# thodan/epos

Measured on AMD Instinct MI355X. Metric: images/sec end-to-end (CNN+PnP-RANSAC), YCB-V 640x480, higher is better.
Workload: dtype f32

## Files before the change

epos_amd/_lib.py:

```python
import ctypes
import os

from epos_amd import build as _build

c_f32p = ctypes.POINTER(ctypes.c_float)
c_f64p = ctypes.POINTER(ctypes.c_double)
c_i32p = ctypes.POINTER(ctypes.c_int32)
c_i64p = ctypes.POINTER(ctypes.c_int64)
c_u64p = ctypes.POINTER(ctypes.c_uint64)
vp = ctypes.c_void_p


class EposError(RuntimeError):
  pass


class PointwiseArgs(ctypes.Structure):
  _fields_ = [
      ('A', vp), ('lda', ctypes.c_int64),
      ('Wp', vp), ('bias', vp),
      ('R', vp), ('ldr', ctypes.c_int64),
      ('C', vp), ('ldc', ctypes.c_int64),
      ('M', ctypes.c_int32), ('N', ctypes.c_int32), ('K', ctypes.c_int32),
      ('relu', ctypes.c_int32), ('relu_in', ctypes.c_int32),
# ... 137 lines not shown
      ('use_prosac', ctypes.c_int32),
      ('lo_iters', ctypes.c_int32),
      ('gc_sweeps', ctypes.c_int32),
      ('pearl_iters', ctypes.c_int32),
  ]


class PnpRansacParams(ctypes.Structure):
  _fields_ = [
      ('iterations_count', ctypes.c_int32),
      ('min_point_number', ctypes.c_int32),
      ('reprojection_error', ctypes.c_double),
      ('confidence', ctypes.c_double),
  ]


SYMBOLS = {
    'epos_abi_version': (ctypes.c_int, []),
    'epos_last_error': (ctypes.c_char_p, []),
    'epos_device_count': (ctypes.c_int, []),
    'epos_clock_probe': (ctypes.c_int, [ctypes.c_void_p, ctypes.c_int, ctypes.c_void_p]),
    'epos_pack_pointwise_weights': (ctypes.c_int64,
                                    [vp, ctypes.c_int, ctypes.c_int, vp]),
    'epos_pack_pointwise_weights_split': (ctypes.c_int64,
                                          [vp, ctypes.c_int, ctypes.c_int, vp]),
    'epos_pack_pointwise_weights_h2': (ctypes.c_int64,
                                       [vp, ctypes.c_int, ctypes.c_int, vp]),
    'epos_absmax_f32': (ctypes.c_int, [vp, ctypes.c_int64, ctypes.c_int64,
                                       ctypes.c_int64, vp, vp]),
    'epos_amax_clear': (ctypes.c_int, [vp, ctypes.c_int64, vp]),
    'epos_pointwise_conv_f32': (ctypes.c_int,
                                [ctypes.POINTER(PointwiseArgs), vp]),
    'epos_pointwise_conv_grouped_f32': (ctypes.c_int, [
        ctypes.POINTER(PointwiseArgs), ctypes.c_int, vp]),
    'epos_conv3x3_f32': (ctypes.c_int, [ctypes.POINTER(Conv3x3Args), ctypes.c_void_p]),
    'epos_depthwise3x3_f32': (ctypes.c_int,
                              [ctypes.POINTER(DepthwiseArgs), vp]),
    'epos_separable_conv_f32': (ctypes.c_int, [ctypes.POINTER(SepConvArgs), vp]),
    'epos_set_h2_narrow_tile_limit': (ctypes.c_int, [ctypes.c_int]),
    'epos_im2col3x3_f32': (ctypes.c_int, [ctypes.POINTER(Im2colArgs), vp]),
    'epos_im2col_f32': (ctypes.c_int, [ctypes.POINTER(Im2colKArgs), vp]),
    'epos_global_avg_pool_partial_f32': (ctypes.c_int, [
        vp, ctypes.c_int64, vp, ctypes.c_int, ctypes.c_int, ctypes.c_int, ctypes.c_int, vp]),
    'epos_global_avg_pool_f32': (ctypes.c_int, [
        vp, ctypes.c_int64, vp, ctypes.c_int, ctypes.c_int, ctypes.c_int, vp]),
    'epos_resize_bilinear_f32': (ctypes.c_int, [
        vp, ctypes.c_int64, vp, ctypes.c_int64, ctypes.c_int, ctypes.c_int,
        ctypes.c_int, ctypes.c_int, ctypes.c_int, ctypes.c_int, vp]),
    'epos_maxpool3x3_s2_f32': (ctypes.c_int, [
        vp, ctypes.c_int64, vp, ctypes.c_int64, ctypes.c_int, ctypes.c_int,
        ctypes.c_int, ctypes.c_int, vp]),
    'epos_subsample_f32': (ctypes.c_int, [
        vp, ctypes.c_int64, vp, ctypes.c_int64, ctypes.c_int, ctypes.c_int,
        ctypes.c_int, ctypes.c_int, ctypes.c_int, vp]),
    'epos_add_relu_f32': (ctypes.c_int, [vp, vp, vp, ctypes.c_int64, vp]),
    'epos_softmax_groups_f32': (ctypes.c_int,
                                [vp, ctypes.c_int64, ctypes.c_int, vp]),
    'epos_u8_to_f32': (ctypes.c_int, [vp, vp, ctypes.c_int64, vp]),
    'epos_scatter_blocks_f32': (ctypes.c_int, [vp, vp, vp, ctypes.c_int64, ctypes.c_int, vp]),
    'epos_argmax_i64': (ctypes.c_int, [
        vp, ctypes.c_int64, vp, ctypes.c_int64, ctypes.c_int, vp]),
    'epos_softmax_slots_f32': (ctypes.c_int, [
        vp, vp, ctypes.c_int, ctypes.c_int, ctypes.c_int, ctypes.c_int, vp]),
    'epos_corr_count': (ctypes.c_int, [
        vp, vp, vp, ctypes.c_int, ctypes.c_int, ctypes.c_int, ctypes.c_int,
        ctypes.c_int, ctypes.c_float, ctypes.c_float, vp, vp, vp, vp, vp]),
# ... 100 lines not shown
```

epos_amd/csrc/pointwise_gemm.h:

```cpp
#pragma once
#include <stdlib.h>

#include <mutex>
#include <type_traits>

#include "common.h"

namespace epos {

struct Fp32MfmaRef {
  int (*dma)(const EposPointwiseArgs* args, int count, hipStream_t s, const int* conv_cin,
             const int* conv_rate);
  int (*staged)(const EposPointwiseArgs* args, int count, hipStream_t s);
};
Fp32MfmaRef& fp32_mfma_ref();
int launch_grouped_split(const EposPointwiseArgs* args, int count, hipStream_t s,
                         const int* conv_cin = nullptr, const int* conv_rate = nullptr);
bool split_eligible(const EposPointwiseArgs* args, int count);
int launch_grouped_h2(const EposPointwiseArgs* args, int count, hipStream_t s,
                      const int* conv_cin = nullptr, const int* conv_rate = nullptr);
bool h2_eligible(const EposPointwiseArgs* args, int count);

namespace {

struct LdsAttrOnce {
  std::mutex mu;
  bool set[16] = {};
};
inline int ensure_dynamic_lds(LdsAttrOnce& once, const void* kern, int bytes, const char* what) {
  int dev = 0;
  if (hipGetDevice(&dev) != hipSuccess || dev < 0 || dev >= 16) {
    set_error("%s: no current device", what);
    return EPOS_E_INVALID;
  }
  std::lock_guard<std::mutex> lock(once.mu);
  if (once.set[dev]) return EPOS_OK;
  const int rc = check_hip(hipFuncSetAttribute(kern, hipFuncAttributeMaxDynamicSharedMemorySize,
                                               bytes), what);
  if (!rc) once.set[dev] = true;
  return rc;
}

constexpr int BN = 128;
constexpr int BK = 32;
constexpr int LDS_A_ROW = BK + 4;
constexpr int LDS_B_TILE = (BK / 4) * BN * 4;
constexpr int THREADS = 256;
constexpr int MAX_GROUP = 8;

typedef float f32x16 __attribute__((ext_vector_type(16)));

struct GroupedArgs {
  EposPointwiseArgs p[MAX_GROUP];
  int tile_start[MAX_GROUP + 1];
// ... 135 lines not shown
```

epos_amd/csrc/pointwise_gemm.hip:

```cpp
#include "pointwise_gemm.h"

namespace epos {

Fp32MfmaRef& fp32_mfma_ref() {
  static Fp32MfmaRef hooks = {nullptr, nullptr};
  return hooks;
}

namespace {

int no_fp32_mfma(const char* what) {
  set_error("%s: this problem brings neither fp16-pair (Wh + a bound for A) nor bf16 x 6 (Ws) "
            "weights, and this build of libepos_hip.so carries no fp32-MFMA kernel (they are "
            "test-only since round 6: libepos_hip_ref.so, `python -m epos_amd.build --ref`, "
            "EPOS_HIP_LIB=<that file>)", what);
  return EPOS_E_INVALID;
}

constexpr int GEMV_SLICES = 16;

__global__ __launch_bounds__(64 * GEMV_SLICES) void pointwise_gemv_f32(EposPointwiseArgs p,
                                                                       int npad) {
  __shared__ float part[GEMV_SLICES][64];
  const int t = threadIdx.x;
// ... 73 lines not shown
  const int64_t npad = round_up(N, BN);
  const int64_t total = kg * npad * 4;
  if (!dst) return total;
  for (int64_t q = 0; q < kg; ++q)
    for (int64_t n = 0; n < npad; ++n)
      for (int e = 0; e < 4; ++e) {
        const int64_t k = q * 4 + e;
        dst[(q * npad + n) * 4 + e] =
            (k < K && n < N) ? w_kn[k * static_cast<int64_t>(N) + n] : 0.f;
      }
  return total;
}

static int grouped_impl(const EposPointwiseArgs* args, int count, void* stream);

extern "C" int epos_pointwise_conv_grouped_f32(const EposPointwiseArgs* args,
                                               int count, void* stream) {
  using namespace epos;
  EPOS_REQUIRE(args && count >= 1 && count <= MAX_GROUP, "1..8 problems per group");
  for (int i = 0; i < count; ++i) {
    const EposPointwiseArgs& a = args[i];
    EPOS_REQUIRE(a.reserved0 == 0, "EposPointwiseArgs.reserved0 must be 0 (ABI 7)");
    if (a.col_sums)
      EPOS_REQUIRE(!a.R && a.N % 4 == 0 && a.col_ld % 4 == 0 && a.col_ld >= a.N &&
                       (reinterpret_cast<uintptr_t>(a.col_sums) & 15) == 0 &&
                       (a.ldc & 3) == 0 && (reinterpret_cast<uintptr_t>(a.C) & 15) == 0 &&
                       h2_eligible(args, count),
                   "col_sums needs the fp16-pair kernel (Wh, a bound for A), no residual, "
                   "N, ldc, col_ld multiples of 4 and 16-byte aligned C / col_sums");
  }
  return grouped_impl(args, count, stream);
}

static int grouped_impl(const EposPointwiseArgs* args, int count, void* stream) {
  using namespace epos;
  hipStream_t s = static_cast<hipStream_t>(stream);
  for (int i = 0; i < count; ++i) {
    const int rc = validate(&args[i]);
    if (rc) return rc;
    EPOS_REQUIRE((args[i].relu_in != 0) == (args[0].relu_in != 0) &&
                 (args[i].R != nullptr) == (args[0].R != nullptr),
                 "problems of one group must agree on relu_in / residual");
  }
  if (count == 1 && args[0].M <= 8 && args[0].sub == 1) {
    const int npad = static_cast<int>(round_up(args[0].N, BN));
    hipLaunchKernelGGL(pointwise_gemv_f32, dim3(npad / 64, args[0].M),
                       dim3(64 * GEMV_SLICES), 0, s, args[0], npad);
    return launch_status("pointwise_gemv_f32");
  }
  if (h2_eligible(args, count)) return launch_grouped_h2(args, count, s);
  for (int i = 0; i < count; ++i)
    EPOS_REQUIRE(!args[i].a_presplit,
                 "a pre-split A operand needs the fp16-pair kernel (every problem of the "
                 "group with Wh; EPOS_GEMM_H2 / EPOS_GEMM_SPLIT not 0)");
  if (split_eligible(args, count)) return launch_grouped_split(args, count, s);
  const Fp32MfmaRef& ref = fp32_mfma_ref();
  static const int use_dma = [] {
    const char* e = getenv("EPOS_GEMM_DMA");
    return e ? atoi(e) : -1;
  }();
  if (args[0].relu_in == 0 && use_dma != 0 && ref.dma)
    return ref.dma(args, count, s, nullptr, nullptr);
  if (ref.staged) return ref.staged(args, count, s);
  return no_fp32_mfma("epos_pointwise_conv_grouped_f32");
}

// ... 57 lines not shown
```

epos_amd/csrc/pointwise_gemm_h2.hip:

```cpp
#include <string.h>

#include <mutex>
#include <utility>

#include "h2_scale.h"
#include "pointwise_gemm.h"

namespace epos {
namespace {

typedef _Float16 f16x8 __attribute__((ext_vector_type(8)));
typedef unsigned u32x4 __attribute__((ext_vector_type(4)));
typedef float h2_f32x4 __attribute__((ext_vector_type(4)));

#ifdef EPOS_GEMM_TRACE
__device__ uint64_t* g_h2_trace = nullptr;
#define H2_STAMP(i) do { if (g_h2_trace && t == 0) g_h2_trace[8 * static_cast<uint64_t>(blockIdx.x) + (i)] = wall_clock64(); } while (0)
#else
#define H2_STAMP(i) do { } while (0)
#endif
constexpr int RING_DEVICES = 16;
constexpr int H2_BM = 128, H2_BN = 128, H2_BK = 16;
constexpr int H2_W_BYTES = H2_BK * H2_BN * 4;
constexpr int H2_A_BYTES = H2_BM * H2_BK * 4;
// ... 784 lines not shown
}

void set_tn_div(GroupedArgs& g, int i) {
  const unsigned d = static_cast<unsigned>(g.tiles_n[i] > 0 ? g.tiles_n[i] : 1);
  unsigned l = 0;
  while ((1ull << l) < d) ++l;
  g.tn_mul[i] = static_cast<unsigned>(((1ull << 32) * ((1ull << l) - d)) / d + 1);
  g.tn_sh1[i] = l > 0 ? 1 : 0;
  g.tn_sh2[i] = l > 0 ? l - 1 : 0;
}

constexpr int RING_SLOTS = 256;
unsigned* ring_slot(hipStream_t s) {
  static std::mutex mu;
  static unsigned* base[RING_DEVICES] = {};
  static unsigned next[RING_DEVICES] = {};
  int dev = 0;
  if (hipGetDevice(&dev) != hipSuccess || dev < 0 || dev >= RING_DEVICES) return nullptr;
  {
    std::lock_guard<std::mutex> lock(mu);
    if (!base[dev] && capturing(s)) return nullptr;
    if (!base[dev] &&
        hipMalloc(reinterpret_cast<void**>(&base[dev]),
                  sizeof(unsigned) * EPOS_AMAX_WORDS * RING_SLOTS) != hipSuccess) {
      base[dev] = nullptr;
      return nullptr;
    }
  }
  const unsigned i = __atomic_fetch_add(&next[dev], 1u, __ATOMIC_RELAXED) % RING_SLOTS;
  return base[dev] + static_cast<size_t>(i) * EPOS_AMAX_WORDS;
}

}

bool h2_eligible(const EposPointwiseArgs* args, int count) {
  static const int mode = [] {
    const char* e = getenv("EPOS_GEMM_H2");
    const char* sp = getenv("EPOS_GEMM_SPLIT");
    if (sp && atoi(sp) == 0) return 0;
    return e ? atoi(e) : 1;
  }();
  if (mode == 0) return false;
  for (int i = 0; i < count; ++i) {
    const EposPointwiseArgs& a = args[i];
    if (!a.Wh || a.relu_in != 0 || a.M <= 8 || (a.K & 3) != 0 || (a.lda & 3) != 0 ||
        (reinterpret_cast<uintptr_t>(a.A) & 15) != 0)
      return false;
    if (a.a_presplit && !a.a_amax) return false;
    const int64_t rows = a.sub > 1 ? static_cast<int64_t>(a.M) / (static_cast<int64_t>(a.Ho) * a.Wo) *
                                         a.Hi * a.Wi
                                   : a.M;
    if (rows * a.lda * 4 >= (1LL << 32)) return false;
  }
  return true;
}

int& narrow_limit() {
  static int v = [] {
    const char* e = getenv("EPOS_H2_BN64_MAX_TILES");
    return e ? atoi(e) : 100;
  }();
  return v;
}

int launch_grouped_h2(const EposPointwiseArgs* args, int count, hipStream_t s,
                      const int* conv_cin, const int* conv_rate) {
// ... 220 lines not shown
```

epos_amd/net.py:

```python
import ctypes
import os

import numpy as np
import torch

from epos_amd import _lib
from epos_amd import weights as W
from epos_amd.net_modes import Bf16Mode, Fp32Mode, _ptr

XCEPTION_BN_EPS = 1e-3
HEAD_BN_EPS = 1e-5
RESNET_BN_EPS = 1e-5
MODES = {'fp32': Fp32Mode, 'bf16': Bf16Mode}
PRECISIONS = tuple(MODES)
PREPROCESS = {None: _lib.PREPROCESS_NONE, 'unit_range': _lib.PREPROCESS_UNIT_RANGE,
              'sub_mean': _lib.PREPROCESS_SUB_MEAN}
PREPROCESS_EXPR = {'unit_range': 'preprocess(input)', 'sub_mean': 'submean(input)'}


def scale_dimension(dim, scale):
  return int((float(dim) - 1.0) * scale + 1.0)


_CAPTURE_STREAMS = {}
# ... 407 lines not shown
    mode.resize('decoder/resize', proj, 256, dcat, ldd, eh, ew, dh, dw_, 256)
    self._set_expr(dcat, self._expr_of(proj) if (eh, ew) == (dh, dw_) else
                   'resize(%s,%dx%d)' % (self._expr_of(proj), dh, dw_), 0, 256)
    m_dec = B * dh * dw_
    self._conv1x1('decoder/feature_projection0', HEAD_BN_EPS, ll, 0, lc, m_dec, lc, dcat,
                  256, ldd, relu=True)
    mode.concat_bound(dcat, proj)
    self.decoder_concat = dcat[..., :304]
    x, c = dcat, 304
    for j in range(2):
      scope = 'decoder/decoder_conv%d' % j
      d, _, _ = self._depthwise(scope + '_depthwise', x, self._ld(x), dh, dw_, c, 1, 1,
                                HEAD_BN_EPS, False, True)
      y = self._abuf(B, dh, dw_, 256)
      self._conv1x1(scope + '_pointwise', HEAD_BN_EPS, d, 0, self._ld(d), m_dec, c, y, 0,
                    256, relu=True)
      x, c = y, 256
    self.decoder_out = x
    self.out_h, self.out_w = dh, dw_

    self.logits = {}
    grp = []
    self._n_trunk_ops = len(self.ops)
    for name, ch in sorted(W.outputs_to_num_channels(
        self.num_objs, self.num_frags).items()):
      buf = self._empty(B, dh, dw_, ch)
      self._conv1x1('logits/' + name, None, x, 0, 256, m_dec, 256, buf, 0, ch, relu=False,
                    group=grp, track_out=False)
      self.logits[name] = buf
    if os.environ.get('EPOS_HEAD_NT_STORES', '1') == '1':
      for g in grp:
        g[1].c_stream = 1
    oname, oargs, oflops = [g for g in grp if g[0].endswith(W.PRED_OBJ_CONF)][0][:3]
    mode.flush(grp)
    self._obj_head_op = (oname, mode.obj_head(oname, oargs))
    self._obj_head_flops = oflops
    self._decoder_x = x

    obj = self.logits[W.PRED_OBJ_CONF]
    frag = self.logits[W.PRED_FRAG_CONF]
    self.obj_label = self._empty(B, dh, dw_, dtype=torch.int64)
    O, F = self.num_objs, self.num_frags
    softmax = self._fn('epos_softmax_groups_f32')
    self.post_ops = [
        ('softmax_obj', self._call('softmax_obj', softmax, (_ptr(obj), m_dec, O + 1))),
        ('softmax_frag', self._call('softmax_frag', softmax, (_ptr(frag), m_dec * O, F))),
        ('argmax', self._call('argmax', self._fn('epos_argmax_i64'),
                              (_ptr(obj), O + 1, _ptr(self.obj_label), m_dec, O + 1)))]
    eo = self._expr_of(self.logits[W.PRED_OBJ_CONF])
    ef = self._expr_of(self.logits[W.PRED_FRAG_CONF])
    el = self._expr_of(self.logits[W.PRED_FRAG_LOC])
    self.trace_outputs = {
        W.PRED_OBJ_CONF: {'expr': 'softmax(%s)' % eo, 'shape': [B, dh, dw_, O + 1]},
        W.PRED_OBJ_LABEL: {'expr': 'argmax(softmax(%s))' % eo, 'shape': [B, dh, dw_]},
        W.PRED_FRAG_CONF: {'expr': 'softmax(reshape(%s,%s))' % (ef, [O, F]),
                           'shape': [B, dh, dw_, O, F]},
        W.PRED_FRAG_LOC: {'expr': 'reshape(%s,%s)' % (el, [O, F, 3]),
                          'shape': [B, dh, dw_, O, F, 3]}}
    mode.finish()

  def algorithmic_bytes(self, dense_heads=True):
    total = self._glue_bytes
    for a_bytes, rest, a_id in self.op_io.values():
      total += self._dw_reads.get(a_id, a_bytes) + rest
    if not dense_heads:
      total -= 4 * self.B * self.out_h * self.out_w * (4 * self.num_objs * self.num_frags)
    return total
# ... 151 lines not shown
```

epos_amd/net_modes.py:

```python
import ctypes
import os

import numpy as np
import torch

from epos_amd import _lib
from epos_amd import weights as W


def _ptr(t, offset_elems=0):
  return ctypes.c_void_p(t.data_ptr() + offset_elems * t.element_size())


def _fold(w_kn, scale, kmult):
  k, n = w_kn.shape
  w = w_kn.astype(np.float32) * scale[None, :].astype(np.float32)
  kpad = -(-k // kmult) * kmult
  if kpad != k:
    w = np.concatenate([w, np.zeros((kpad - k, n), np.float32)], 0)
  return np.ascontiguousarray(w)


def _pack(fn, w, dtype):
  src = w.ctypes.data_as(ctypes.c_void_p)
  total = fn(src, w.shape[0], w.shape[1], None)
  if total <= 0:
    return None
  dst = np.empty(total, dtype)
  fn(src, w.shape[0], w.shape[1], dst.ctypes.data_as(ctypes.c_void_p))
  return dst


def _bias(bias, n, mult):
  b = np.zeros(-(-n // mult) * mult, np.float32)
  b[:n] = bias
  return b


class Fp32Mode(object):

  dtype, line = torch.float32, 32
  MAX_SLOTS = 512

  def __init__(self, net):
    self.net = net
    fn = net._fn
    self.gemm = fn('epos_pointwise_conv_grouped_f32')
    self.gemm1 = fn('epos_pointwise_conv_f32')
    self.dw = fn('epos_depthwise3x3_f32')
    self.conv3x3 = fn('epos_conv3x3_f32')
    self.im2col3x3 = fn('epos_im2col3x3_f32')
    self.im2col_k = fn('epos_im2col_f32')
    self.absmax = fn('epos_absmax_f32')
    self.amax_clear = fn('epos_amax_clear')
    self.avg_pool = fn('epos_global_avg_pool_f32')
    self.avg_pool_partial = fn('epos_global_avg_pool_partial_f32')
    self.resize_fn = fn('epos_resize_bilinear_f32')
    self.subsample = fn('epos_subsample_f32')
    self.add_relu = fn('epos_add_relu_f32')
    self.maxpool = fn('epos_maxpool3x3_s2_f32')
    self.pack_plain = fn('epos_pack_pointwise_weights')
    self.pack_split = fn('epos_pack_pointwise_weights_split')
    self.pack_h2 = fn('epos_pack_pointwise_weights_h2')
    self._amax_table = torch.zeros(self.MAX_SLOTS * _lib.AMAX_WORDS, dtype=torch.int32,
                                   device=net.dev)
    self._slot_count = ctypes.c_int64(0)
    self._bounds = {}
    self.use_h2 = (os.environ.get('EPOS_GEMM_H2', '1') != '0' and
                   os.environ.get('EPOS_GEMM_SPLIT', '1') != '0')
    self.use_presplit = self.use_h2 and os.environ.get('EPOS_H2_PRESPLIT', '1') == '1'
    self._dw_h2 = {}
    self.h2_layers, self.h2_refused, self.presplit_layers = [], [], []
    self._last_pw = None
    self._first_im2col = None

  @property
  def _n_slots(self):
    return self._slot_count.value

  def _new_slot(self):
    i = self._slot_count.value
# ... 66 lines not shown
                ldr=0, sub=1, ho=0, wo=0, hi=0, wi=0, group=None, track_out=True):
    net = self.net
    ab = self._bounds.get(id(a)) if self.use_h2 else None
    wp, bp, ws, wh, kpad = self._weights(name, conv, ab is not None and m > 8)
    n = conv[0].shape[1]
    assert kpad == k or (kpad > k and lda >= kpad), (name, k, kpad, lda)
    dwa = self._dw_h2.pop(id(a), None)
    presplit = False
    if dwa is not None:
      presplit = wh is not None and sub == 1 and a_off == 0
      dwa.y_h2 = int(presplit)
      if presplit:
        self.presplit_layers.append(name)
    track = track_out and m > 8 and (res is None or ldr % 4 == 0)
    cslot = self._out_slot(c, n, ldc, c_off) if track else None
    h = wh is not None
    args = _lib.PointwiseArgs(
        A=_ptr(a, a_off), lda=lda, Wp=_ptr(wp), bias=_ptr(bp),
        R=_ptr(res, res_off) if res is not None else None, ldr=ldr,
        C=_ptr(c, c_off), ldc=ldc, M=m, N=n, K=kpad, relu=int(relu), sub=sub,
        Ho=ho, Wo=wo, Hi=hi, Wi=wi, Ws=_ptr(ws), Wh=_ptr(wh) if h else None,
        a_amax=self._slot_ptr(ab[0]) if h else None,
        a_amax2=self._slot_ptr(ab[1]) if h else None,
        a_gain=ab[2] if h else 0.0, a_bias=ab[3] if h else 0.0,
        a_presplit=int(presplit), c_amax=self._slot_ptr(cslot))
    nbytes = 4 * (m * k + k * n + m * n + (m * n if res is not None else 0))
    net.op_io[name] = (4 * m * k, nbytes - 4 * m * k, id(a))
    if group is not None:
      group.append((name, args, 2 * m * n * k, nbytes))
      return
    net._launch(name, self.gemm, (args, 1), 'gemm', 2 * m * n * k, nbytes)
    self._last_pw = (c, args, h and res is None and c_off == 0 and n % 4 == 0)

  def flush(self, group):
    for kind in sorted({g[1].a_presplit for g in group}):
      part = [g for g in group if g[1].a_presplit == kind]
      arr = (_lib.PointwiseArgs * len(part))(*[g[1] for g in part])
      self.net._launch('+'.join(g[0] for g in part), self.gemm, (arr, len(part)), 'gemm',
                       sum(g[2] for g in part), sum(g[3] for g in part))
    del group[:]

  def depthwise(self, name, x, y, gain, bias0, flops, nbytes, **fields):
    xb = self._bounds.get(id(x))
    if xb is not None:
      self._set_bound(y, xb[0], xb[1], gain * (xb[2] if xb[2] else 1.0), gain * xb[3] + bias0)
    args = _lib.DepthwiseArgs(**fields)
    yb = self._bounds.get(id(y))
    if yb is not None and self.use_presplit:
      args.y_h2 = 1
      args.x_amax, args.x_amax2 = self._slot_ptr(yb[0]), self._slot_ptr(yb[1])
      args.gain, args.bias0 = yb[2], yb[3]
      self._dw_h2[id(y)] = args
    self.net._launch(name, self.dw, (args,), 'dw', flops, nbytes)

  def dense_conv(self, name, x, y, hi, wi, cin, ho, wo, kk, stride, rate, pad, preprocess,
                 conv):
    net, B = self.net, self.net.B
    cout = y.shape[3]
    k = kk * kk * cin
    if kk == 3 and cin % 32 == 0 and preprocess == _lib.PREPROCESS_NONE:
      xb = self._bounds.get(id(x))
      wp, bp, ws, wh, _ = self._weights(name, conv, xb is not None and xb[1] is None and
                                        xb[2] == 0.0)
      yslot = self._out_slot(y, cout, cout)
      args = _lib.Conv3x3Args(X=_ptr(x), ldx=cin, Wp=_ptr(wp), bias=_ptr(bp), Y=_ptr(y),
                              ldy=cout, B=B, H=hi, W=wi, Cin=cin, Cout=cout, stride=stride,
                              rate=rate, relu=1, Ws=_ptr(ws),
                              Wh=_ptr(wh) if wh is not None else None,
                              x_amax=self._slot_ptr(xb[0]) if wh is not None else None,
                              y_amax=self._slot_ptr(yslot))
      net._launch(name, self.conv3x3, (args,), 'gemm', 2 * B * ho * wo * cout * k,
# ... 134 lines not shown
    args = _lib.PointwiseBf16Args(
        A=_ptr(a, a_off) if a is not None else None, lda=lda, Wp=_ptr(wp), bias=_ptr(bp),
        R=_ptr(res, res_off) if res is not None else None, ldr=ldr,
        C=_ptr(c, c_off), ldc=ldc, M=m, N=n, K=kpad, relu=int(relu), sub=sub,
        Ho=ho, Wo=wo, Hi=hi, Wi=wi, c_f32=int(c.dtype == torch.float32), c_stream=0)
    nbytes = (2 * (m * k + k * n) + c.element_size() * m * n +
              (2 * m * n if res is not None else 0))
    net.op_io[name] = (2 * m * k, nbytes - 2 * m * k, id(a))
    if group is not None:
      group.append((name, args, 2 * m * n * k, nbytes))
      return args
    net._launch(name, self.gemm, (args, 1), 'gemm', 2 * m * n * k, nbytes)
    return args

  def _pointwise_f32(self, name, a, lda, m, k, conv, c, ldc, relu):
    net = self.net
    w_kn, scale, bias = conv
    n = w_kn.shape[1]
    kpad = -(-k // 4) * 4
    assert kpad == k, (name, k)
    if net.dry_run:
      wp, bp, ws = net._empty(1), net._empty(1), net._empty(1)
    else:
      w = _fold(w_kn, scale, 4)
      wp, bp = net._dev(_pack(self.pack_plain, w, np.float32)), net._dev(_bias(bias, n, 128))
      ws = net._dev(_pack(self.pack_split, w, np.uint8))
    args = _lib.PointwiseArgs(A=_ptr(a), lda=lda, Wp=_ptr(wp), bias=_ptr(bp), C=_ptr(c),
                              ldc=ldc, M=m, N=n, K=kpad, relu=int(relu), sub=1, Ws=_ptr(ws))
    nbytes = 4 * (m * k + k * n + m * n)
    net.op_io[name] = (4 * m * k, nbytes - 4 * m * k, id(a))
    net._launch(name, self.gemm_f32, (args, 1), 'gemm', 2 * m * n * k, nbytes)
    return args

  def flush(self, group):
    if group:
      arr = (_lib.PointwiseBf16Args * len(group))(*[g[1] for g in group])
      self.net._launch('+'.join(g[0] for g in group), self.gemm, (arr, len(group)), 'gemm',
                       sum(g[2] for g in group), sum(g[3] for g in group))
    del group[:]

  def depthwise(self, name, x, y, gain, bias0, flops, nbytes, **fields):
    self.net._launch(name, self.dw, (_lib.DepthwiseBf16Args(**fields),), 'dw', flops, nbytes)

  def dense_conv(self, name, x, y, hi, wi, cin, ho, wo, kk, stride, rate, pad, preprocess,
                 conv):
    net, B = self.net, self.net.B
    k = kk * kk * cin
    ldcol = -(-k // 8) * 8
    m = B * ho * wo
    self._col_elems = max(self._col_elems, m * ldcol)
    args = _lib.Im2colBf16Args(
        X=_ptr(x), ldx=cin, x_bf16=int(x.dtype == torch.bfloat16), col=None, ldcol=ldcol,
        B=B, Hi=hi, Wi=wi, Ho=ho, Wo=wo, C=cin, k=kk, stride=stride, rate=rate, pad=pad,
        preprocess=preprocess, mean_rgb=(ctypes.c_float * 3)(*W.MEAN_RGB))
    self._col_users.append((args, 'col'))
    net._launch(name + '/im2col', self.im2col, (args,), 'im2col')
    gargs = self.pointwise(name, None, 0, ldcol, m, k, conv, y, 0, y.shape[3], relu=True)
    self._col_users.append((gargs, 'A'))
    net.op_io[name] = (x.element_size() * B * hi * wi * cin, net.op_io[name][1], id(x))

  def mean(self, name, x, pooled, hw, c):
    self.net._launch(name, self.avg_pool, (_ptr(x), c, _ptr(pooled), self.net.B, hw, c))
    return False

  def resize(self, name, x, ldx, y, ldy, hi, wi, ho, wo, c):
    self.net._launch(name, self.resize_fn, (_ptr(x), ldx, int(x.dtype == torch.float32),
                                            _ptr(y), ldy, self.net.B, hi, wi, ho, wo, c))
# ... 25 lines not shown
```

include/epos_hip.h:

```cpp
#ifndef EPOS_HIP_H_
#define EPOS_HIP_H_

#include <stdint.h>

#ifdef __cplusplus
extern "C" {
#endif

#define EPOS_OK 0
#define EPOS_E_INVALID (-1)
#define EPOS_E_CAPACITY (-2)
#define EPOS_E_NODEVICE (-3)
#define EPOS_E_INTERNAL (-4)
#define EPOS_E_HIP_BASE (-1000)

#define EPOS_ABI_VERSION 7

int epos_abi_version(void);
const char* epos_last_error(void);
int epos_device_count(void);
int epos_clock_probe(int64_t* out2, int microseconds, void* stream);


int64_t epos_pack_pointwise_weights(const float* w_kn, int K, int N, float* dst);
// ... 4 lines not shown

#define EPOS_AMAX_WORDS 64
int epos_absmax_f32(const float* X, int64_t ldx, int64_t rows, int64_t cols,
                    uint32_t* slot, void* stream);
int epos_amax_clear(uint32_t* slots, int64_t n_slots, void* stream);

typedef struct EposPointwiseArgs {
  const float* A; int64_t lda;
  const float* Wp; const float* bias;
  const float* R; int64_t ldr;
  float* C; int64_t ldc;
  int32_t M, N, K;
  int32_t relu;
  int32_t relu_in;
  int32_t sub;
  int32_t Ho, Wo, Hi, Wi;
  const void* Ws;
  const void* Wh;
  const uint32_t* a_amax;
  const uint32_t* a_amax2;
  float a_gain, a_bias;
  int32_t a_presplit;
  uint32_t* c_amax;
  float* col_sums;
  int64_t col_ld;
  int32_t c_stream;
  int32_t reserved0;
} EposPointwiseArgs;
int epos_pointwise_conv_f32(const EposPointwiseArgs* args, void* stream);

int epos_pointwise_conv_grouped_f32(const EposPointwiseArgs* args, int count,
                                    void* stream);


typedef struct EposConv3x3Args {
  const float* X; int64_t ldx;
  const float* Wp; const float* bias;
  float* Y; int64_t ldy;
  int32_t B, H, W, Cin, Cout;
  int32_t stride, rate;
  int32_t relu;
  const void* Ws;
  const void* Wh;
  const uint32_t* x_amax;
  uint32_t* y_amax;
} EposConv3x3Args;
int epos_conv3x3_f32(const EposConv3x3Args* args, void* stream);

typedef struct EposDepthwiseArgs {
  const float* X; int64_t ldx;
  const float* w9c; const float* bias;
  float* Y; int64_t ldy;
  int32_t B, Hi, Wi, Ho, Wo, C;
  int32_t stride, rate;
  int32_t relu_in, relu_out;
  int32_t y_h2;
  const uint32_t* x_amax;
  const uint32_t* x_amax2;
  float gain, bias0;
} EposDepthwiseArgs;
int epos_depthwise3x3_f32(const EposDepthwiseArgs* args, void* stream);

int epos_set_h2_narrow_tile_limit(int max_tiles);
typedef struct EposSepConvArgs {
  EposDepthwiseArgs dw;
  EposPointwiseArgs pw;
// ... 207 lines not shown
```

Measured before the change: 387.8.

## Add specialized fp16-pair GEMM kernel for K=256 decoder prediction heads

Adds a dedicated grouped GEMM kernel for the decoder output heads (K=256). It keeps the split-fp16 A panel in registers across a range of N tiles and streams weights through an 8-stage LDS ring, prefetching the next tile's weights and epilogue operands. Panels are spread across XCD-style groups, and the tile range per block is picked by a cost model. The net routes the head flush through the new kernel by default, falling back to the generic grouped path when ineligible. This adds complexity and register pressure, and assumes that register reuse of A outweighs the lower per-block parallelism.

New measurement: 394.1 (median of 6 runs). 1.02x the previous value.

```diff
diff --git a/epos_amd/_lib.py b/epos_amd/_lib.py
--- a/epos_amd/_lib.py
+++ b/epos_amd/_lib.py
@@ -193,6 +193,8 @@
     'epos_pointwise_conv_f32': (ctypes.c_int,
                                 [ctypes.POINTER(PointwiseArgs), vp]),
     'epos_pointwise_conv_grouped_f32': (ctypes.c_int, [
+        ctypes.POINTER(PointwiseArgs), ctypes.c_int, vp]),
+    'epos_heads_gemm_f32': (ctypes.c_int, [
         ctypes.POINTER(PointwiseArgs), ctypes.c_int, vp]),
     'epos_conv3x3_f32': (ctypes.c_int, [ctypes.POINTER(Conv3x3Args), ctypes.c_void_p]),
     'epos_depthwise3x3_f32': (ctypes.c_int,
diff --git a/epos_amd/csrc/heads_gemm_h2.hip b/epos_amd/csrc/heads_gemm_h2.hip
--- /dev/null
+++ b/epos_amd/csrc/heads_gemm_h2.hip
@@ -0,0 +1,367 @@
+#include "h2_scale.h"
+#include "pointwise_gemm.h"
+
+namespace epos {
+namespace {
+
+typedef _Float16 hd_f16x8 __attribute__((ext_vector_type(8)));
+typedef unsigned hd_u32x4 __attribute__((ext_vector_type(4)));
+
+constexpr int HD_BM = 128, HD_BN = 64, HD_BK = 16;
+constexpr int HD_K = 256;
+constexpr int HD_NKS = HD_K / HD_BK;
+constexpr int HD_NS = 8;
+constexpr int HD_LA = HD_NS - 1;
+constexpr int HD_STAGE = 4 * 1024;
+constexpr int HD_RING = HD_NS * HD_STAGE;
+constexpr int HD_OPS = 2 * 4 * 1024;
+constexpr int HD_EPR = HD_BN + 4;
+constexpr int HD_EPI = 4 * 32 * HD_EPR * 4;
+constexpr int HD_LDS = HD_RING + HD_OPS + HD_EPI;
+constexpr int HD_S_MIN = 8;
+constexpr unsigned HD_OOB = 0x80000000u;
+static_assert(HD_NKS % HD_NS == 0, "stage of a K step = its index mod HD_NS");
+static_assert(HD_LA - 2 + 2 + HD_S_MIN <= 63, "vmcnt is a 6-bit counter");
+
+struct HeadsArgs {
+  EposPointwiseArgs p[MAX_GROUP];
+  int tile0[MAX_GROUP + 1];
+  int count;
+  int nt;
+  int panels;
+  int range;
+  int nr;
+  const float* zero_chunk;
+};
+
+template <int... I, class F>
+__device__ __forceinline__ void hd_static_for(std::integer_sequence<int, I...>, F&& f) {
+  (f(std::integral_constant<int, I>{}), ...);
+}
+template <int N> __device__ __forceinline__ void hd_wait_vm_lgkm0() {
+  asm volatile("s_waitcnt vmcnt(%0) lgkmcnt(0)" : : "n"(N) : "memory");
+}
+__device__ __forceinline__ void glds4_v_m0(const float* gsrc, unsigned lds_dst) {
+  asm volatile("s_mov_b32 m0, %1\n\ts_nop 0\n\tglobal_load_lds_dword %0, off"
+               : : "v"(gsrc), "s"(lds_dst) : "memory", "m0");
+}
+
+struct HdTile {
+  const float* w;
+  const float* cn;
+  const float* bias;
+  int n0, N, pi;
+};
+__device__ __forceinline__ HdTile hd_tile(const HeadsArgs* gp, int t) {
+  int pi = 0;
+#pragma unroll
+  for (int i = 1; i < MAX_GROUP; ++i)
+    if (i < gp->count && t >= gp->tile0[i]) pi = i;
+  const EposPointwiseArgs& q = gp->p[pi];
+  const int tl = t - gp->tile0[pi];
+  const int tn128 = (q.N + 127) >> 7;
+  const char* wh = static_cast<const char*>(q.Wh);
+  HdTile r;
+  r.w = reinterpret_cast<const float*>(wh + static_cast<int64_t>(tl >> 1) * HD_NKS * 8192 +
+                                       (tl & 1) * 4096);
+  r.cn = reinterpret_cast<const float*>(wh + static_cast<int64_t>(tn128) * HD_NKS * 8192) +
+         tl * HD_BN;
+  r.bias = q.bias;
+  r.n0 = tl * HD_BN;
+  r.N = q.N;
+  r.pi = pi;
+  return r;
+}
+
+__device__ __forceinline__ void hd_mfma(const hd_u32x4& a, const hd_u32x4& b, f32x16& c) {
+  c = __builtin_amdgcn_mfma_f32_32x32x16_f16(__builtin_bit_cast(hd_f16x8, a),
+                                             __builtin_bit_cast(hd_f16x8, b), c, 0, 0, 0);
+}
+
+__global__ __launch_bounds__(256, 2) void heads_gemm_h2_f32(HeadsArgs ga_) {
+  (void)ga_;
+  const HeadsArgs* __restrict__ gp = (const HeadsArgs*)__builtin_amdgcn_kernarg_segment_ptr();
+  extern __shared__ __attribute__((aligned(16))) float smem[];
+  const int t = threadIdx.x;
+  const int lane = t & 63;
+  const int wave = t >> 6;
+  const int wave_u = __builtin_amdgcn_readfirstlane(wave);
+  const int l31 = lane & 31, h = lane >> 5;
+
+  int panel, t0, t1;
+  {
+    const int raw = blockIdx.x, x = raw & 7, k = raw >> 3;
+    const int P = gp->panels;
+    const int p_lo = (x * P) >> 3, p_hi = ((x + 1) * P) >> 3;
+    const int px = p_hi - p_lo;
+    if (k >= px * gp->nr) return;
+    const int r = k / px;
+    panel = p_lo + (k - r * px);
+    t0 = r * gp->range;
+    t1 = t0 + gp->range < gp->nt ? t0 + gp->range : gp->nt;
+  }
+  const EposPointwiseArgs& pa = gp->p[0];
+  const int M = pa.M;
+  const int m0 = panel * HD_BM;
+  const float* zero_chunk = gp->zero_chunk;
+
+  unsigned am_raw = 0, am_raw2 = 0;
+  h2_scale_load(pa.a_amax, pa.a_amax2, lane, am_raw, am_raw2);
+
+  const unsigned lds0 = static_cast<unsigned>(reinterpret_cast<uintptr_t>(
+      (__attribute__((address_space(3))) float*)smem));
+  const unsigned w_voff = static_cast<unsigned>(wave * 1024 + lane * 16);
+  const unsigned w_dst = lds0 + wave_u * 1024;
+  const unsigned ops_dst = lds0 + HD_RING + wave_u * 1024;
+
+  auto issue_w = [&](const HdTile& ti, int kq, int slot) {
+    glds16_s_m0(w_voff, uniform_ptr(ti.w + kq * (8192 / 4)), w_dst + slot * HD_STAGE);
+  };
+  auto issue_ops = [&](const HdTile& ti, int par) {
+    glds4_v_m0(ti.cn + lane, ops_dst + par * 4096);
+    const int n = ti.n0 + lane;
+    const float* b = (ti.bias && n < ti.N) ? ti.bias + n : zero_chunk;
+    glds4_v_m0(b, ops_dst + par * 4096 + 256);
+  };
+
+  HdTile cur = hd_tile(gp, t0);
+  HdTile nxt = hd_tile(gp, t0 + 1 < t1 ? t0 + 1 : t0);
+  hd_u32x4 ah[HD_NKS], am[HD_NKS];
+  float inv_a;
+  {
+    int m = m0 + wave * 32 + l31;
+    m = m < M ? m : M - 1;
+    const float* arow = pa.A + static_cast<int64_t>(m) * pa.lda + 8 * h;
+    float4 xa[2 * HD_NKS];
+#pragma unroll
+    for (int ks = 0; ks < HD_NKS; ++ks) {
+      xa[2 * ks] = *reinterpret_cast<const float4*>(arow + ks * HD_BK);
+      xa[2 * ks + 1] = *reinterpret_cast<const float4*>(arow + ks * HD_BK + 4);
+    }
+    issue_w(cur, 0, 0);
+    issue_ops(cur, 0);
+#pragma unroll
+    for (int q = 1; q < HD_LA; ++q) issue_w(cur, q, q);
+    float sa_v, inv_a_v;
+    h2_scale_finish(am_raw, am_raw2, pa.a_gain, pa.a_bias, sa_v, inv_a_v);
+    const float sa = __uint_as_float(__builtin_amdgcn_readfirstlane(__float_as_uint(sa_v)));
+    inv_a = __uint_as_float(__builtin_amdgcn_readfirstlane(__float_as_uint(inv_a_v)));
+#pragma unroll
+    for (int ks = 0; ks < HD_NKS; ++ks)
+#pragma unroll
+      for (int u = 0; u < 4; ++u) {
+        const float4 x4 = xa[2 * ks + (u >> 1)];
+        const float x0 = (u & 1) ? x4.z : x4.x, x1 = (u & 1) ? x4.w : x4.y;
+        unsigned hh, mm;
+        h2_split_pair(x0, x1, sa, hh, mm);
+        ah[ks][u] = hh;
+        am[ks][u] = mm;
+      }
+  }
+
+  hd_wait_vm_lgkm0<2 + HD_LA - 1>();
+  __builtin_amdgcn_s_barrier();
+  const int b_off = lane * 4;
+  hd_u32x4 bp[2][2];
+#pragma unroll
+  for (int cb = 0; cb < 2; ++cb)
+#pragma unroll
+    for (int pc = 0; pc < 2; ++pc)
+      bp[cb][pc] = *reinterpret_cast<const hd_u32x4*>(smem + b_off + (cb * 2 + pc) * 256);
+
+  float* ws = smem + (HD_RING + HD_OPS) / 4 + wave * 32 * HD_EPR;
+  const int c4 = lane & 15, r0 = lane >> 4;
+
+  for (int tt = t0; tt < t1; ++tt) {
+    const bool first = tt == t0;
+    const int par = (tt - t0) & 1;
+    f32x16 acc[2], corr[2];
+#pragma unroll
+    for (int j = 0; j < 2; ++j)
+#pragma unroll
+      for (int r = 0; r < 16; ++r) { acc[j][r] = 0.f; corr[j][r] = 0.f; }
+
+    auto step = [&](auto ks_tag) {
+      constexpr int ks = decltype(ks_tag)::value;
+      constexpr int younger = (HD_LA - 2) + (ks >= 10 ? 2 : 0);
+      static_assert(HD_LA == 7, "the counts above are written for 7 steps ahead");
+      if constexpr (ks <= 5) {
+        if (first) hd_wait_vm_lgkm0<younger>();
+        else hd_wait_vm_lgkm0<younger + HD_S_MIN>();
+      } else {
+        hd_wait_vm_lgkm0<younger>();
+      }
+      __builtin_amdgcn_s_barrier();
+      constexpr int s1 = (ks + 1) % HD_NS;
+      hd_u32x4 nb[2][2];
+#pragma unroll
+      for (int cb = 0; cb < 2; ++cb)
+#pragma unroll
+        for (int pc = 0; pc < 2; ++pc)
+          nb[cb][pc] = *reinterpret_cast<const hd_u32x4*>(smem + s1 * (HD_STAGE / 4) + b_off +
+                                                          (cb * 2 + pc) * 256);
+      __builtin_amdgcn_sched_barrier(0);
+      hd_mfma(ah[ks], bp[0][1], corr[0]);
+      __builtin_amdgcn_sched_barrier(0);
+      {
+        constexpr int q = ks + HD_LA;
+        constexpr int slot = q % HD_NS;
+        if constexpr (q < HD_NKS) issue_w(cur, q, slot);
+        else issue_w(nxt, q - HD_NKS, slot);
+      }
+      __builtin_amdgcn_sched_barrier(0);
+      hd_mfma(ah[ks], bp[1][1], corr[1]);
+      if constexpr (ks + HD_LA == HD_NKS) {
+        __builtin_amdgcn_sched_barrier(0);
+        issue_ops(nxt, par ^ 1);
+        __builtin_amdgcn_sched_barrier(0);
+      }
+      hd_mfma(am[ks], bp[0][0], corr[0]);
+      hd_mfma(am[ks], bp[1][0], corr[1]);
+      hd_mfma(ah[ks], bp[0][0], acc[0]);
+      hd_mfma(ah[ks], bp[1][0], acc[1]);
+#pragma unroll
+      for (int cb = 0; cb < 2; ++cb) { bp[cb][0] = nb[cb][0]; bp[cb][1] = nb[cb][1]; }
+    };
+    hd_static_for(std::make_integer_sequence<int, HD_NKS>{}, step);
+
+#pragma unroll
+    for (int j = 0; j < 2; ++j)
+#pragma unroll
+      for (int r = 0; r < 16; ++r)
+        ws[((r & 3) + 8 * (r >> 2) + 4 * h) * HD_EPR + j * 32 + l31] =
+            __builtin_fmaf(corr[j][r], 0x1p-11f, acc[j][r]);
+    __builtin_amdgcn_fence(__ATOMIC_RELEASE, "wavefront");
+    const float* ops = smem + (HD_RING + par * 4096) / 4 + wave * 256;
+    const float4 cn4 = *reinterpret_cast<const float4*>(ops + c4 * 4);
+    const float4 b4 = *reinterpret_cast<const float4*>(ops + 64 + c4 * 4);
+    float4 v[8];
+#pragma unroll
+    for (int i = 0; i < 8; ++i) {
+      v[i] = *reinterpret_cast<const float4*>(ws + (r0 + 4 * i) * HD_EPR + c4 * 4);
+      v[i].x = v[i].x * cn4.x * inv_a + b4.x;
+      v[i].y = v[i].y * cn4.y * inv_a + b4.y;
+      v[i].z = v[i].z * cn4.z * inv_a + b4.z;
+      v[i].w = v[i].w * cn4.w * inv_a + b4.w;
+    }
+    const EposPointwiseArgs& q = gp->p[cur.pi];
+    const int rows = M - m0 < HD_BM ? M - m0 : HD_BM;
+    const int64_t ldc = q.ldc;
+    const __amdgpu_buffer_rsrc_t rsrc = __builtin_amdgcn_make_buffer_rsrc(
+        q.C + static_cast<int64_t>(m0) * ldc, 0, static_cast<int>(rows * ldc * 4), 0x00020000);
+    const int n = cur.n0 + c4 * 4;
+    const unsigned row0 = static_cast<unsigned>(wave * 32 + r0);
+    const bool vec = (ldc & 3) == 0 && (cur.N & 3) == 0 &&
+                     (reinterpret_cast<uintptr_t>(q.C) & 15) == 0;
+    auto opaque = [](unsigned x) { asm volatile("" : "+v"(x)); return x; };
+    if (vec) {
+      const unsigned oob = n < cur.N ? 0u : HD_OOB;
+      const unsigned nb4 = static_cast<unsigned>(n) * 4u;
+#pragma unroll
+      for (int i = 0; i < 8; ++i) {
+        const int off = static_cast<int>(
+            opaque(((row0 + 4 * i) * static_cast<unsigned>(ldc) * 4u + nb4) | oob));
+        if (q.c_stream)
+          __builtin_amdgcn_raw_buffer_store_b128(__builtin_bit_cast(hd_u32x4, v[i]), rsrc, off, 0, 2);
+        else
+          __builtin_amdgcn_raw_buffer_store_b128(__builtin_bit_cast(hd_u32x4, v[i]), rsrc, off, 0, 0);
+      }
+    } else {
+#pragma unroll
+      for (int i = 0; i < 8; ++i) {
+        const float e4[4] = {v[i].x, v[i].y, v[i].z, v[i].w};
+#pragma unroll
+        for (int e = 0; e < 4; ++e) {
+          const unsigned oob = n + e < cur.N ? 0u : HD_OOB;
+          const int off = static_cast<int>(opaque(
+              (((row0 + 4 * i) * static_cast<unsigned>(ldc) + static_cast<unsigned>(n + e)) * 4u) |
+              oob));
+          __builtin_amdgcn_raw_buffer_store_b32(__float_as_uint(e4[e]), rsrc, off, 0, 0);
+        }
+      }
+    }
+    cur = nxt;
+    nxt = hd_tile(gp, tt + 2 < t1 ? tt + 2 : t1 - 1);
+  }
+  asm volatile("s_waitcnt vmcnt(0)" ::: "memory");
+}
+
+int choose_range(int nt, int panels, int cus) {
+  const int slots = cus > 8 ? cus * 2 / 8 : 1;
+  const int pmax = (panels + 7) / 8;
+  int best = nt < 4 ? nt : 4;
+  int64_t best_cost = -1;
+  for (int r = 4; r <= 32; ++r) {
+    const int rr = r < nt ? r : nt;
+    const int64_t nr = (nt + rr - 1) / rr;
+    const int64_t rounds = (pmax * nr + slots - 1) / slots;
+    const int64_t cost = rounds * (rr + 1);
+    if (best_cost < 0 || cost < best_cost) { best_cost = cost; best = rr; }
+    if (rr == nt) break;
+  }
+  return best;
+}
+
+int device_cus() {
+  static int cus[16] = {};
+  int dev = 0;
+  if (hipGetDevice(&dev) != hipSuccess || dev < 0 || dev >= 16) return 256;
+  int n = __atomic_load_n(&cus[dev], __ATOMIC_RELAXED);
+  if (n > 0) return n;
+  if (hipDeviceGetAttribute(&n, hipDeviceAttributeMultiprocessorCount, dev) != hipSuccess || n <= 0)
+    n = 256;
+  __atomic_store_n(&cus[dev], n, __ATOMIC_RELAXED);
+  return n;
+}
+
+}
+
+bool heads_eligible(const EposPointwiseArgs* args, int count) {
+  if (count < 1 || count > MAX_GROUP) return false;
+  const EposPointwiseArgs& a0 = args[0];
+  if (!a0.a_amax) return false;
+  for (int i = 0; i < count; ++i) {
+    const EposPointwiseArgs& a = args[i];
+    if (a.A != a0.A || a.lda != a0.lda || a.M != a0.M || a.K != HD_K || a.sub != 1 ||
+        a.R || a.relu || a.relu_in || a.a_presplit || a.c_amax || a.col_sums || !a.Wh ||
+        a.a_amax != a0.a_amax || a.a_amax2 != a0.a_amax2 || a.a_gain != a0.a_gain ||
+        a.a_bias != a0.a_bias || a.N < 1 || a.M < 1 || a.ldc < a.N ||
+        a.ldc > (1LL << 20) ||
+        (reinterpret_cast<uintptr_t>(a.Wh) & 15) != 0 ||
+        (reinterpret_cast<uintptr_t>(a.bias) & 3) != 0)
+      return false;
+  }
+  return true;
+}
+
+int launch_heads_h2(const EposPointwiseArgs* args, int count, const float* zero_chunk,
+                    hipStream_t s) {
+  HeadsArgs g = {};
+  g.count = count;
+  int nt = 0;
+  for (int i = 0; i < count; ++i) {
+    g.p[i] = args[i];
+    g.tile0[i] = nt;
+    nt += static_cast<int>(ceil_div(args[i].N, HD_BN));
+  }
+  for (int i = count; i <= MAX_GROUP; ++i) g.tile0[i] = nt;
+  g.nt = nt;
+  g.panels = static_cast<int>(ceil_div(args[0].M, HD_BM));
+  g.range = choose_range(nt, g.panels, device_cus());
+  g.nr = static_cast<int>(ceil_div(nt, g.range));
+  g.zero_chunk = zero_chunk;
+  int items = 0;
+  for (int x = 0; x < 8; ++x) {
+    const int px = ((x + 1) * g.panels >> 3) - (x * g.panels >> 3);
+    items = px * g.nr > items ? px * g.nr : items;
+  }
+  if (items <= 0) return EPOS_OK;
+  static LdsAttrOnce once;
+  const int rc = ensure_dynamic_lds(once, reinterpret_cast<const void*>(heads_gemm_h2_f32),
+                                    HD_LDS, "hipFuncSetAttribute(heads_gemm_h2_f32)");
+  if (rc) return rc;
+  hipLaunchKernelGGL(heads_gemm_h2_f32, dim3(8 * items), dim3(256), HD_LDS, s, g);
+  return launch_status("heads_gemm_h2_f32");
+}
+
+}
diff --git a/epos_amd/csrc/pointwise_gemm.h b/epos_amd/csrc/pointwise_gemm.h
--- a/epos_amd/csrc/pointwise_gemm.h
+++ b/epos_amd/csrc/pointwise_gemm.h
@@ -20,6 +20,10 @@
 int launch_grouped_h2(const EposPointwiseArgs* args, int count, hipStream_t s,
                       const int* conv_cin = nullptr, const int* conv_rate = nullptr);
 bool h2_eligible(const EposPointwiseArgs* args, int count);
+bool heads_eligible(const EposPointwiseArgs* args, int count);
+int launch_heads_h2(const EposPointwiseArgs* args, int count, const float* zero_chunk,
+                    hipStream_t s);
+const float* h2_zero_chunk(hipStream_t s);
 
 namespace {
 
diff --git a/epos_amd/csrc/pointwise_gemm.hip b/epos_amd/csrc/pointwise_gemm.hip
--- a/epos_amd/csrc/pointwise_gemm.hip
+++ b/epos_amd/csrc/pointwise_gemm.hip
@@ -129,6 +129,23 @@
   return grouped_impl(args, count, stream);
 }
 
+extern "C" int epos_heads_gemm_f32(const EposPointwiseArgs* args, int count, void* stream) {
+  using namespace epos;
+  EPOS_REQUIRE(args && count >= 1 && count <= MAX_GROUP, "1..8 problems per group");
+  if (!h2_eligible(args, count) || !heads_eligible(args, count))
+    return epos_pointwise_conv_grouped_f32(args, count, stream);
+  for (int i = 0; i < count; ++i) {
+    EPOS_REQUIRE(args[i].reserved0 == 0, "EposPointwiseArgs.reserved0 must be 0 (ABI 7)");
+    const int rc = validate(&args[i]);
+    if (rc) return rc;
+  }
+  hipStream_t s = static_cast<hipStream_t>(stream);
+  const float* z = h2_zero_chunk(s);
+  EPOS_REQUIRE(z, "cannot allocate the zero chunk (first fp16-pair launch on this device "
+                  "during a stream capture? launch once before capturing)");
+  return launch_heads_h2(args, count, z, s);
+}
+
 static int grouped_impl(const EposPointwiseArgs* args, int count, void* stream) {
   using namespace epos;
   hipStream_t s = static_cast<hipStream_t>(stream);
diff --git a/epos_amd/csrc/pointwise_gemm_h2.hip b/epos_amd/csrc/pointwise_gemm_h2.hip
--- a/epos_amd/csrc/pointwise_gemm_h2.hip
+++ b/epos_amd/csrc/pointwise_gemm_h2.hip
@@ -840,6 +840,8 @@
 }
 
 }
+
+const float* h2_zero_chunk(hipStream_t s) { return zero_chunk_dev(s); }
 
 bool h2_eligible(const EposPointwiseArgs* args, int count) {
   static const int mode = [] {
diff --git a/epos_amd/net.py b/epos_amd/net.py
--- a/epos_amd/net.py
+++ b/epos_amd/net.py
@@ -463,7 +463,7 @@
       for g in grp:
         g[1].c_stream = 1
     oname, oargs, oflops = [g for g in grp if g[0].endswith(W.PRED_OBJ_CONF)][0][:3]
-    mode.flush(grp)
+    mode.flush(grp, heads=os.environ.get('EPOS_HEADS_KERNEL', '1') == '1')
     self._obj_head_op = (oname, mode.obj_head(oname, oargs))
     self._obj_head_flops = oflops
     self._decoder_x = x
diff --git a/epos_amd/net_modes.py b/epos_amd/net_modes.py
--- a/epos_amd/net_modes.py
+++ b/epos_amd/net_modes.py
@@ -47,6 +47,7 @@
     fn = net._fn
     self.gemm = fn('epos_pointwise_conv_grouped_f32')
     self.gemm1 = fn('epos_pointwise_conv_f32')
+    self.heads = fn('epos_heads_gemm_f32')
     self.dw = fn('epos_depthwise3x3_f32')
     self.conv3x3 = fn('epos_conv3x3_f32')
     self.im2col3x3 = fn('epos_im2col3x3_f32')
@@ -179,11 +180,12 @@
     net._launch(name, self.gemm, (args, 1), 'gemm', 2 * m * n * k, nbytes)
     self._last_pw = (c, args, h and res is None and c_off == 0 and n % 4 == 0)
 
-  def flush(self, group):
+  def flush(self, group, heads=False):
     for kind in sorted({g[1].a_presplit for g in group}):
       part = [g for g in group if g[1].a_presplit == kind]
       arr = (_lib.PointwiseArgs * len(part))(*[g[1] for g in part])
-      self.net._launch('+'.join(g[0] for g in part), self.gemm, (arr, len(part)), 'gemm',
+      fn = self.heads if heads and not kind else self.gemm
+      self.net._launch('+'.join(g[0] for g in part), fn, (arr, len(part)), 'gemm',
                        sum(g[2] for g in part), sum(g[3] for g in part))
     del group[:]
 
@@ -384,7 +386,7 @@
     net._launch(name, self.gemm_f32, (args, 1), 'gemm', 2 * m * n * k, nbytes)
     return args
 
-  def flush(self, group):
+  def flush(self, group, heads=False):
     if group:
       arr = (_lib.PointwiseBf16Args * len(group))(*[g[1] for g in group])
       self.net._launch('+'.join(g[0] for g in group), self.gemm, (arr, len(group)), 'gemm',
diff --git a/include/epos_hip.h b/include/epos_hip.h
--- a/include/epos_hip.h
+++ b/include/epos_hip.h
@@ -60,6 +60,8 @@
 int epos_pointwise_conv_grouped_f32(const EposPointwiseArgs* args, int count,
                                     void* stream);
 
+int epos_heads_gemm_f32(const EposPointwiseArgs* args, int count, void* stream);
+
 
 typedef struct EposConv3x3Args {
   const float* X; int64_t ldx;
```
